# HSoumi/hybrid-als-twotower-recommender

Hardware: NVIDIA B200
Metric: als_ratings_per_sec_per_sweep (higher is better)
Workload: dtype f32

## Files before the change

### hybrid-als-twotower-recommender_b200/csrc/als_ws64.cu

```cuda
#include <cuda_bf16.h>

#include <cstdlib>

#include "als_ws_common.cuh"

namespace hals {
namespace ws64 {
using namespace ws;

constexpr int K = 64;
constexpr int kStageBytes = stage_bytes(K);
#ifndef HALS_WS_STAGES
#define HALS_WS_STAGES 10
#endif
constexpr int kStages = HALS_WS_STAGES;
constexpr int kAcc = 4, kAccCols = 128;
constexpr int kSlots = 2;
constexpr int kLd = 68;
constexpr int kSlotBytes = 2 * 64 * kLd * 4 + 512;
constexpr int kSolvers = 9;
constexpr int kScratchBytes = 1536;
constexpr int kN = 80;
constexpr int kThreads = 512;
constexpr int kWarpSolver = 0, kWarpGather = 9, kWarpMma = 11, kWarpDrain = 12;
static_assert(kStages % 2 == 0, "the two gather warps own alternate stages");
static_assert(kWarpSolver + kSolvers == kWarpGather && kWarpDrain + 4 == kThreads / 32 && kWarpDrain % 4 == 0, "role map");

struct Bars {
  uint64_t st_full[kStages], st_free[kStages];
  uint64_t st_scaled[kStages];
  uint64_t acc_full[kAcc], acc_free[kAcc];
  uint64_t sol_full[kSolvers];
  uint64_t slot_free[kSlots];
};

__device__ __forceinline__ float sel4(float a, float b, float c, float d, int i) {
  return i == 0 ? a : i == 1 ? b : i == 2 ? c : d;
}

__device__ __noinline__ void gather_role(uint32_t stages, Bars* bars, uint8_t* gscratch, const Range* rg,
                                         const int32_t* __restrict__ colidx, const uint32_t* __restrict__ vals_hl,
                                         const float* __restrict__ vals_sc, const uint8_t* __restrict__ src_hl, int zero_row,
                                         const int64_t* __restrict__ chunk_pos, const int32_t* __restrict__ chunk_cnt,
                                         int gw, int lane) {
  const int t_sub = lane >> 4, piece = lane & 15;
  const uint32_t ring = umma::smem_u32(gscratch);
  const uint32_t mpos = ring + 2 * kBurst * 128;
  const uint32_t mcnt = mpos + 2 * kBurst * 8;
  const int64_t k_hi = rg->chunk_hi;
  int64_t kw = rg->chunk_lo + gw;
  auto load_window = [&](int64_t& p, int& c) {
    const int64_t k = kw + 2 * lane;
    p = 0; c = 0;
    if (k < k_hi) { p = __ldg(chunk_pos + k); c = __ldg(chunk_cnt + k); }
    kw += 64;
  };
  int64_t wpos, npos;
  int wcnt, ncnt;
  load_window(wpos, wcnt);
  load_window(npos, ncnt);
  int wb = 0;
  int ci[kBurst];
  auto fill = [&](int buf) {
    if (lane >= wb * kBurst && lane < (wb + 1) * kBurst) {
      const uint32_t e = (uint32_t)(buf * kBurst + lane - wb * kBurst);
      asm volatile("st.shared.b64 [%0], %1;\n" ::"r"(mpos + e * 8u), "l"(wpos) : "memory");
      asm volatile("st.shared.b32 [%0], %1;\n" ::"r"(mcnt + e * 4u), "r"(wcnt) : "memory");
    }
#pragma unroll
    for (int c = 0; c < kBurst; ++c) {
      const int64_t pos = __shfl_sync(0xffffffffu, wpos, wb * kBurst + c);
      const int cnt = __shfl_sync(0xffffffffu, wcnt, wb * kBurst + c);
      ci[c] = lane < cnt ? __ldg(colidx + pos + lane) : zero_row;
    }
    if (++wb == 32 / kBurst) {
      wb = 0;
      wpos = npos; wcnt = ncnt;
      load_window(npos, ncnt);
    }
  };
  auto stash = [&](int buf) {
#pragma unroll
    for (int c = 0; c < kBurst; ++c)
      sts32(ring + (uint32_t)((buf * kBurst + c) * 32 + (lane & 1) * 16 + (lane >> 1)) * 4u, __int_as_float(ci[c]));
    __syncwarp();
  };

  const uint32_t blk_off = piece < 8 ? 0u : (uint32_t)kBlk;
  uint32_t dsto[4];
#pragma unroll
  for (int i = 0; i < 4; ++i) {
    const int t = t_sub + 2 * i;
    dsto[i] = blk_off + (uint32_t)t * kRowBytes + (uint32_t)(((piece & 7) ^ (t & 7)) << 4);
  }
  const uint64_t srcb = reinterpret_cast<uint64_t>(src_hl) + (uint64_t)piece * 16u;
  const uint32_t rdst = 2 * kBlk + (uint32_t)lane * kRowBytes + (uint32_t)((lane & 7) << 4);
  const uint32_t sdst = 2 * kBlk + (uint32_t)lane * kRowBytes + (uint32_t)((7 ^ (lane & 7)) << 4);
  uint32_t g = 0, s = (uint32_t)gw, u = 0;
#ifdef HALS_WS_PROFILE
  long long w_free = 0, t_iss = 0, t_fill = 0;
#endif
  fill(0);
  stash(0);
  fill(1);
  for (int buf = 0;; buf ^= 1) {
    bool done = false;
#pragma unroll 1
    for (int c = 0; c < kBurst; ++c) {
      int cnt;
      asm volatile("ld.shared.b32 %0, [%1];\n" : "=r"(cnt) : "r"(mcnt + (uint32_t)(buf * kBurst + c) * 4u));
      if (cnt <= 0) { done = true; break; }
      int64_t pos;
      asm volatile("ld.shared.b64 %0, [%1];\n" : "=l"(pos) : "r"(mpos + (uint32_t)(buf * kBurst + c) * 8u));
      const uint32_t ir = ring + (uint32_t)((buf * kBurst + c) * 32 + t_sub * 16) * 4u;
      const float4 c0 = lds128(ir), c1 = lds128(ir + 16), c2 = lds128(ir + 32), c3 = lds128(ir + 48);
      if (u > 0) { WS_T0(); umma::mbar_wait(&bars->st_free[s], (u - 1) & 1); WS_ACC(w_free); }
      WS_T0();
      const uint32_t st = stages + s * kStageBytes;
      const float colf[16] = {c0.x, c0.y, c0.z, c0.w, c1.x, c1.y, c1.z, c1.w, c2.x, c2.y, c2.z, c2.w, c3.x, c3.y, c3.z, c3.w};
#pragma unroll
      for (int i = 0; i < KC / 2; ++i) {
        uint64_t src;
        asm("mad.wide.u32 %0, %1, 256, %2;\n" : "=l"(src) : "r"((uint32_t)__float_as_int(colf[i])), "l"(srcb));
        cp_async16_raw(st + dsto[i & 3] + (uint32_t)(i >> 2) * (8 * kRowBytes), src);
      }
      {
        const bool ok = lane < cnt;
        const uint32_t* rp = vals_hl + pos + (ok ? lane : 0);
        asm volatile("cp.async.ca.shared.global [%0], [%1], 4, %2;\n" ::"r"(st + rdst), "l"(rp), "r"(ok ? 4 : 0) : "memory");
        if (vals_sc != nullptr) {
          const float* sp = vals_sc + pos + (ok ? lane : 0);
          asm volatile("cp.async.ca.shared.global [%0], [%1], 4, %2;\n" ::"r"(st + sdst), "l"(sp), "r"(ok ? 4 : 0) : "memory");
        }
      }
      cp_async_mbar_arrive_noinc(&bars->st_full[s]);
      WS_ACC(t_iss);
      ++g;
      s += 2;
      if (s >= (uint32_t)kStages) { s -= kStages; ++u; }
    }
    if (done) break;
    WS_T0();
    stash(buf ^ 1);
    fill(buf);
    WS_ACC(t_fill);
  }
#ifdef HALS_WS_PROFILE
  if (lane == 0 && blockIdx.x == 1) printf("G%d: chunks %u wait_free %lld issue %lld fill %lld\n", gw, g, w_free, t_iss, t_fill);
#endif
}

__device__ __noinline__ void scaler_role(uint32_t stages, Bars* bars, const Range* rg, int lane) {
  scale_stages<K, kStages>(stages, bars, rg, lane);
}

__device__ __noinline__ void mma_role(uint32_t sbase, uint32_t tmem, Bars* bars, const Range* rg,
                                      const int32_t* __restrict__ chunk_cnt, bool scaled, int lane) {
  constexpr uint32_t idesc = umma::make_instr_desc(umma::kFmtBF16, true, true, 128, kN);
  uint64_t* const ready = scaled ? bars->st_scaled : bars->st_full;
  const int64_t k_lo = rg->chunk_lo, k_hi = rg->chunk_hi;
  uint32_t s = 0, su = 0, b = 0, bu = 0;
  bool first = true;
#ifdef HALS_WS_PROFILE
  long long w_acc = 0, w_full = 0, t_issue = 0;
#endif
  int wc = 0, nc = 0;
  if (k_lo + lane < k_hi) wc = __ldg(chunk_cnt + k_lo + lane);
  if (k_lo + 32 + lane < k_hi) nc = __ldg(chunk_cnt + k_lo + 32 + lane);
  const bool leader = elect_one();
  const uint64_t ad0 = umma::make_smem_desc(sbase, kBlk, 1024, umma::kSwizzle128B);
  const uint64_t bd0 = umma::make_smem_desc(sbase, 2 * kBlk, 1024, umma::kSwizzle128B);
  for (int64_t kb = k_lo; kb < k_hi; kb += 32) {
    const int nk = (int)(k_hi - kb < 32 ? k_hi - kb : 32);
    for (int i = 0; i < nk; ++i) {
      const int cnt = __shfl_sync(0xffffffffu, wc, i);
      if (leader) {
        if (first) {
          if (bu > 0) { WS_T0(); umma::mbar_wait(&bars->acc_free[b], (bu - 1) & 1); WS_ACC(w_acc); }
          umma::fence_after_sync();
        }
        { WS_T0(); umma::mbar_wait(&ready[s], su & 1); WS_ACC(w_full); }
        WS_T0();
        const uint32_t td = tmem + b * kAccCols;
        const uint64_t so = (uint64_t)((s * kStageBytes) >> 4);
#pragma unroll
        for (int ks = 0; ks < KC / 16; ++ks)
          umma::mma_bf16(td, ad0 + so + (uint64_t)(ks * 2048 >> 4), bd0 + so + (uint64_t)(ks * 2048 >> 4), idesc,
                         !(first && ks == 0));
        umma::commit(&bars->st_free[s]);
        if (cnt <= KC) umma::commit(&bars->acc_full[b]);
        WS_ACC(t_issue);
      }
      __syncwarp();
      first = cnt <= KC;
      if (first) { if (++b == (uint32_t)kAcc) { b = 0; ++bu; } }
      if (++s == (uint32_t)kStages) { s = 0; ++su; }
    }
    wc = nc;
    nc = 0;
    if (kb + 64 + lane < k_hi) nc = __ldg(chunk_cnt + kb + 64 + lane);
  }
#ifdef HALS_WS_PROFILE
  if (blockIdx.x == 1 && leader) printf("M: wait_acc_free %lld wait_stage_full %lld issue %lld\n", w_acc, w_full, t_issue);
#endif
}

__device__ __noinline__ void drain_role(uint32_t slots, uint32_t tmem, Bars* bars, const Range* rg, int nsolv, int tid) {
  const int warp = tid >> 5;
  const int64_t n_rows = rg->item_hi - rg->item_lo;
  uint32_t b = 0, bu = 0, sl = 0, slu = 0, sv = 0;
#ifdef HALS_WS_PROFILE
  long long w_acc = 0, w_slot = 0, t_ld = 0;
#endif
  for (int64_t it = 0; it < n_rows; ++it) {
    { WS_T0(); umma::mbar_wait(&bars->acc_full[b], bu & 1); WS_ACC(w_acc); }
    umma::fence_after_sync();
    const uint32_t ta = tmem + b * kAccCols + ((uint32_t)(warp * 32) << 16);
    float a[64], e[16];
    {
      WS_T0();
      umma::tmem_ld32(ta, a);
      umma::tmem_ld32(ta + 32, a + 32);
      umma::tmem_ld16(ta + 64, e);
      WS_ACC(t_ld);
    }
    umma::fence_before_sync();
    umma::mbar_arrive(&bars->acc_free[b]);
    if (slu > 0) { WS_T0(); umma::mbar_wait(&bars->slot_free[sl], (slu - 1) & 1); WS_ACC(w_slot); }
    const uint32_t sb = slots + sl * kSlotBytes;
    const int m = tid & 63;
    const uint32_t rowp = sb + (tid < 64 ? 0u : (uint32_t)(64 * kLd * 4)) + (uint32_t)m * (kLd * 4);
#pragma unroll
    for (int n = 0; n < 64; n += 4) sts128(rowp + n * 4, a[n], a[n + 1], a[n + 2], a[n + 3]);
    const uint32_t bp = sb + 2 * 64 * kLd * 4;
    if (tid < 64) sts32(bp + m * 4, e[0] + e[1]);
    else sts32(bp + 256 + m * 4, e[0]);
    umma::mbar_arrive(&bars->sol_full[sv]);
    if (++b == (uint32_t)kAcc) { b = 0; ++bu; }
    if (++sl == (uint32_t)kSlots) { sl = 0; ++slu; }
    if (++sv == (uint32_t)nsolv) sv = 0;
  }
#ifdef HALS_WS_PROFILE
  if (tid == 0 && blockIdx.x == 1) printf("D: wait_acc_full %lld tmem_ld %lld wait_slot_free %lld\n", w_acc, t_ld, w_slot);
#endif
}

template <int JR>
__device__ __forceinline__ void elim_block(f32x2 (&R)[36], f32x2& bb2, const uint32_t P, const uint32_t Y,
                                           const uint32_t DI, const int ti, const int tj, const int lane) {
  const uint32_t oW = (uint32_t)ti * 16u;
  const uint32_t oL = (uint32_t)(tj & 3) * 16u + (uint32_t)(tj >> 2) * 4u;
  const uint32_t oB = oW + (uint32_t)(tj >> 1) * 64u + (uint32_t)(tj & 1) * 8u;
  auto publish = [&](uint32_t Pn, bool own) {
    if (JR & 1) sts64_if(own, Pn + oW + (JR >> 1) * 64 + 8, R[tri(JR, JR)]);
#pragma unroll
    for (int q = (JR + 1) & ~1; q < 8; q += 2) sts128x2_if(own, Pn + oW + (q >> 1) * 64, R[tri(q, JR)], R[tri(q + 1, JR)]);
  };
  {
    publish(P, tj == 0);
    sts32_if(ti == 0 && tj == JR, Y + (uint32_t)(8 * JR) * 4u, lo2(bb2));
    sts32_if(lane == 0, DI + (uint32_t)(8 * JR) * 4u, -rcp_fast(lo2(R[tri(JR, JR)])));
    __syncwarp();
  }
  const bool below = tj > JR;
#pragma unroll 1
  for (int jm = 0; jm < 8; ++jm) {
    const int j = 8 * JR + jm;
    const uint32_t Pj = P + ((uint32_t)(jm & 1) << 8);
    f32x2 w[8];
    float l[8];
    if (JR & 1) w[JR] = lds64x2(Pj + oW + (JR >> 1) * 64 + 8);
#pragma unroll
    for (int q = (JR + 1) & ~1; q < 8; q += 2) lds128x2(Pj + oW + (q >> 1) * 64, w[q], w[q + 1]);
    const float ninv = lds32(DI + (uint32_t)j * 4u);
#pragma unroll
    for (int c = JR; c < 8; ++c) l[c] = lds32(Pj + oL + (c >> 1) * 64 + (c & 1) * 8);
    const float zj = lds32(Y + (uint32_t)j * 4u);
    const f32x2 wb = lds64x2(Pj + oB);
    const f32x2 ninv2 = pack2(ninv, ninv);
    const float lj = tj > jm ? l[JR] : 0.f;
    const f32x2 lj2 = pack2(lj, lj);
    w[JR] = fmul2(w[JR], ninv2);
    R[tri(JR, JR)] = ffma2(w[JR], lj2, R[tri(JR, JR)]);
    const int jn = jm + 1;
    const float ninv_n = -rcp_fast((jn & 4) ? hi2(R[tri(JR, JR)]) : lo2(R[tri(JR, JR)]));
#pragma unroll
    for (int q = JR + 1; q < 8; ++q) {
      w[q] = fmul2(w[q], ninv2);
      R[tri(q, JR)] = ffma2(w[q], lj2, R[tri(q, JR)]);
    }
    {
      const bool on = tj == JR;
      const bool act_lo = below || (on && ti > jm), act_hi = below || (on && ti + 4 > jm);
      const f32x2 mb = fmul2(wb, ninv2);
      bb2 = ffma2(pack2(act_lo ? lo2(mb) : 0.f, act_hi ? hi2(mb) : 0.f), pack2(zj, zj), bb2);
    }
    {
      const uint32_t Pn = P + ((uint32_t)(jn & 1) << 8);
      const bool own = (tj == jn);
      publish(Pn, own);
      sts32_if(tj == JR && ti == (jn & 3) && jn < 8, Y + (uint32_t)(j + 1) * 4u, (jn & 4) ? hi2(bb2) : lo2(bb2));
      sts32_if(own && ti == (jn & 3), DI + (uint32_t)(j + 1) * 4u, ninv_n);
      __syncwarp();
    }
#pragma unroll
    for (int c = JR + 1; c < 8; ++c) {
      const f32x2 l2 = pack2(l[c], l[c]);
#pragma unroll
      for (int q = c; q < 8; ++q) R[tri(q, c)] = ffma2(w[q], l2, R[tri(q, c)]);
    }
  }
}

template <int JR>
__device__ __forceinline__ void back_block(const f32x2 (&R)[36], f32x2 (&x2)[8], const uint32_t Y, const uint32_t DI,
                                           const uint32_t T, const uint32_t RH, const int ti, const int tj,
                                           const int lane, float& out0, float& out1) {
  f32x2 acc0 = 0ull, acc1 = 0ull;
#pragma unroll
  for (int q = JR + 1; q < 8; ++q) {
    if ((q - JR) & 1) acc0 = ffma2(R[tri(q, JR)], x2[q], acc0);
    else acc1 = ffma2(R[tri(q, JR)], x2[q], acc1);
  }
  float ext = (lo2(acc0) + hi2(acc0)) + (lo2(acc1) + hi2(acc1));
  ext += __shfl_xor_sync(0xffffffffu, ext, 8);
  ext += __shfl_xor_sync(0xffffffffu, ext, 16);
  const float rh = lds32(Y + (uint32_t)(8 * JR + tj) * 4u) - ext;
  sts32(T + (uint32_t)(ti * 8 + tj) * 4u, lo2(R[tri(JR, JR)]));
  sts32(T + (uint32_t)((ti + 4) * 8 + tj) * 4u, hi2(R[tri(JR, JR)]));
  sts32_if(ti == 0, RH + (uint32_t)tj * 4u, rh);
  __syncwarp();
  float r[8], di[8], xb[8];
  {
    const float4 a = lds128(RH), b = lds128(RH + 16);
    r[0] = a.x; r[1] = a.y; r[2] = a.z; r[3] = a.w; r[4] = b.x; r[5] = b.y; r[6] = b.z; r[7] = b.w;
    const float4 c = lds128(DI + (uint32_t)(8 * JR) * 4u), d = lds128(DI + (uint32_t)(8 * JR) * 4u + 16);
    di[0] = c.x; di[1] = c.y; di[2] = c.z; di[3] = c.w; di[4] = d.x; di[5] = d.y; di[6] = d.z; di[7] = d.w;
  }
#pragma unroll
  for (int e = 7; e >= 0; --e) {
    xb[e] = -r[e] * di[e];
    if (e > 0) {
      float t[8];
      const float4 a = lds128(T + (uint32_t)(e * 8) * 4u);
      t[0] = a.x; t[1] = a.y; t[2] = a.z; t[3] = a.w;
      if (e > 4) {
        const float4 b = lds128(T + (uint32_t)(e * 8 + 4) * 4u);
        t[4] = b.x; t[5] = b.y; t[6] = b.z; t[7] = b.w;
      }
#pragma unroll
      for (int c = 0; c < e; ++c) r[c] = fmaf(-t[c], xb[e], r[c]);
    }
  }
  __syncwarp();
  x2[JR] = pack2(sel4(xb[0], xb[1], xb[2], xb[3], ti), sel4(xb[4], xb[5], xb[6], xb[7], ti));
  if ((lane >> 2) == JR) {
    const int e2 = lane & 3;
    out0 = sel4(xb[0], xb[2], xb[4], xb[6], e2);
    out1 = sel4(xb[1], xb[3], xb[5], xb[7], e2);
  }
}

__device__ __forceinline__ void eliminate(f32x2 (&R)[36], f32x2& bb2, const uint32_t P, const uint32_t Y, const uint32_t DI,
                                          int ti, int tj, int lane) {
  elim_block<0>(R, bb2, P, Y, DI, ti, tj, lane);
  elim_block<1>(R, bb2, P, Y, DI, ti, tj, lane);
  elim_block<2>(R, bb2, P, Y, DI, ti, tj, lane);
  elim_block<3>(R, bb2, P, Y, DI, ti, tj, lane);
  elim_block<4>(R, bb2, P, Y, DI, ti, tj, lane);
  elim_block<5>(R, bb2, P, Y, DI, ti, tj, lane);
  elim_block<6>(R, bb2, P, Y, DI, ti, tj, lane);
  elim_block<7>(R, bb2, P, Y, DI, ti, tj, lane);
  __syncwarp();
}
__device__ __forceinline__ void back_store(const f32x2 (&R)[36], const uint32_t Y, const uint32_t DI, const uint32_t T,
                                           const uint32_t RH, int ti, int tj, int lane, float* __restrict__ dst,
                                           __nv_bfloat16* __restrict__ dst_hl, int row) {
  f32x2 x2[8];
#pragma unroll
  for (int q = 0; q < 8; ++q) x2[q] = 0ull;
  float out0 = 0.f, out1 = 0.f;
  back_block<7>(R, x2, Y, DI, T, RH, ti, tj, lane, out0, out1);
  back_block<6>(R, x2, Y, DI, T, RH, ti, tj, lane, out0, out1);
  back_block<5>(R, x2, Y, DI, T, RH, ti, tj, lane, out0, out1);
  back_block<4>(R, x2, Y, DI, T, RH, ti, tj, lane, out0, out1);
  back_block<3>(R, x2, Y, DI, T, RH, ti, tj, lane, out0, out1);
  back_block<2>(R, x2, Y, DI, T, RH, ti, tj, lane, out0, out1);
  back_block<1>(R, x2, Y, DI, T, RH, ti, tj, lane, out0, out1);
  back_block<0>(R, x2, Y, DI, T, RH, ti, tj, lane, out0, out1);
  *reinterpret_cast<float2*>(dst + (int64_t)row * K + 2 * lane) = make_float2(out0, out1);
  if (dst_hl) {
    const __nv_bfloat162 h = __floats2bfloat162_rn(out0, out1);
    const __nv_bfloat162 l = __floats2bfloat162_rn(out0 - __low2float(h), out1 - __high2float(h));
    __nv_bfloat162* o = reinterpret_cast<__nv_bfloat162*>(dst_hl + (int64_t)row * (2 * K));
    o[lane] = h;
    o[K / 2 + lane] = l;
  }
}

__device__ __noinline__ void solver_role(uint32_t slots, uint32_t scratch, Bars* bars, float* __restrict__ dst,
                                         __nv_bfloat16* __restrict__ dst_hl, float* __restrict__ workspace, float reg,
                                         const int32_t* __restrict__ item_row, const int32_t* __restrict__ item_len,
                                         const int32_t* __restrict__ item_slot, const float* __restrict__ gram_tiles,
                                         const Range* rg, int nsolv, int w, int lane) {
  const int ti = lane >> 3, tj = lane & 7;
  const uint32_t P = scratch, Y = P + 512, DI = Y + 256, T = DI + 256, RH = T + 256;
  const int64_t n_items = rg->item_hi;
#ifdef HALS_WS_PROFILE
  long long w_slot = 0, t_load = 0, t_elim = 0, t_back = 0;
  int n_solved = 0;
#endif
  int64_t it = rg->item_lo + w;
  int row_n = 0, len_n = 0, slot_n = -1;
  if (it < n_items) { row_n = __ldg(item_row + it); len_n = __ldg(item_len + it); slot_n = __ldg(item_slot + it); }
  uint32_t mine = 0;
  for (uint32_t i = (uint32_t)w; it < n_items; i += nsolv, it += nsolv, ++mine) {
    const int row = row_n, len = len_n, wslot = slot_n;
    {
      const int64_t nx = it + nsolv;
      if (nx < n_items) { row_n = __ldg(item_row + nx); len_n = __ldg(item_len + nx); slot_n = __ldg(item_slot + nx); }
    }
    const uint32_t sl = i % kSlots;
    { WS_T0(); umma::mbar_wait(&bars->sol_full[w], mine & 1); WS_ACC(w_slot); }
    const uint32_t S1 = slots + sl * kSlotBytes, S2 = S1 + 64 * kLd * 4, B1 = S2 + 64 * kLd * 4, B2 = B1 + 256;
    if (wslot >= 0) {
      float* W = workspace + (size_t)wslot * ((size_t)K * K + K + 4);
      for (int e = lane; e < K * K; e += 32) {
        const int m = e >> 6, n = e & 63;
        W[e] = lds32(S1 + (uint32_t)(m * kLd + n) * 4u) + lds32(S2 + (uint32_t)(m * kLd + n) * 4u) +
               lds32(S2 + (uint32_t)(n * kLd + m) * 4u);
      }
      W[K * K + lane] = lds32(B1 + lane * 4) + lds32(B2 + lane * 4);
      W[K * K + 32 + lane] = lds32(B1 + (32 + lane) * 4) + lds32(B2 + (32 + lane) * 4);
      if (lane == 0) W[K * K + K] = (float)len;
      __syncwarp();
      if (lane == 0) umma::mbar_arrive(&bars->slot_free[sl]);
      continue;
    }
    f32x2 R[36];
    f32x2 bb2;
    {
      WS_T0();
      const float lam = reg * (float)len;
      const uint32_t p1 = S1 + (uint32_t)(ti * kLd + tj) * 4u, p2 = S2 + (uint32_t)(ti * kLd + tj) * 4u;
      const uint32_t pt = S2 + (uint32_t)(tj * kLd + ti) * 4u;
#pragma unroll
      for (int q = 0; q < 8; ++q) {
#pragma unroll
        for (int c = 0; c <= q; ++c) {
          float v[2];
#pragma unroll
          for (int h = 0; h < 2; ++h) {
            const uint32_t mn = (uint32_t)((8 * q + 4 * h) * kLd + 8 * c) * 4u, nm = (uint32_t)(8 * c * kLd + 8 * q + 4 * h) * 4u;
            v[h] = lds32(p1 + mn) + lds32(p2 + mn) + lds32(pt + nm);
            if (q == c) v[h] += (ti + 4 * h == tj) ? lam : 0.f;
          }
          R[tri(q, c)] = pack2(v[0], v[1]);
        }
      }
      if (gram_tiles != nullptr) {
        const float4* gp = reinterpret_cast<const float4*>(gram_tiles) + lane * 18;
#pragma unroll
        for (int i = 0; i < 18; ++i) {
          const float4 g = __ldg(gp + i);
          R[2 * i] = ffma2(pack2(g.x, g.y), pack2(1.f, 1.f), R[2 * i]);
          R[2 * i + 1] = ffma2(pack2(g.z, g.w), pack2(1.f, 1.f), R[2 * i + 1]);
        }
      }
      const uint32_t ob = (uint32_t)(ti + 8 * tj) * 4u;
      bb2 = pack2(lds32(B1 + ob) + lds32(B2 + ob), lds32(B1 + ob + 16) + lds32(B2 + ob + 16));
      __syncwarp();
      if (lane == 0) umma::mbar_arrive(&bars->slot_free[sl]);
      WS_ACC(t_load);
    }
    {
      WS_T0();
      eliminate(R, bb2, P, Y, DI, ti, tj, lane);
      WS_ACC(t_elim);
    }
    {
      WS_T0();
      back_store(R, Y, DI, T, RH, ti, tj, lane, dst, dst_hl, row);
      WS_ACC(t_back);
    }
#ifdef HALS_WS_PROFILE
    ++n_solved;
#endif
  }
#ifdef HALS_WS_PROFILE
  if (lane == 0 && blockIdx.x == 1)
    printf("S%d: solved %d wait_slot %lld load %lld elim %lld back %lld\n", w, n_solved, w_slot, t_load, t_elim, t_back);
#endif
}

__global__ void __launch_bounds__(kThreads, 1)
als_ws64_kernel(const int32_t* __restrict__ colidx, const uint32_t* __restrict__ vals_hl,
                const float* __restrict__ vals_sc, const float* __restrict__ gram_tiles,
                const __nv_bfloat16* __restrict__ src_hl, float* __restrict__ dst, float reg,
                const int32_t* __restrict__ item_row, const int32_t* __restrict__ item_len,
                const int32_t* __restrict__ item_slot, const int64_t* __restrict__ item_chunk0,
                const int64_t* __restrict__ item_cost0, const int64_t* __restrict__ chunk_pos,
                const int32_t* __restrict__ chunk_cnt, int64_t n_items, int zero_row, float* __restrict__ workspace,
                __nv_bfloat16* __restrict__ dst_hl) {
  extern __shared__ uint8_t smem_dyn[];
  __shared__ Bars bars;
  __shared__ Range range;
  __shared__ uint32_t tmem_slot;
  uint8_t* base = reinterpret_cast<uint8_t*>((reinterpret_cast<uintptr_t>(smem_dyn) + 1023) & ~uintptr_t(1023));
  const int tid = threadIdx.x, warp = tid >> 5, lane = tid & 31;
  if (warp == kWarpDrain) umma::tmem_alloc(&tmem_slot, kAcc * kAccCols);
  if (tid == 32) {
    for (int s = 0; s < kStages; ++s) {
      umma::mbar_init(&bars.st_full[s], 32);
      umma::mbar_init(&bars.st_free[s], 1);
      umma::mbar_init(&bars.st_scaled[s], 1);
    }
    for (int b = 0; b < kAcc; ++b) { umma::mbar_init(&bars.acc_full[b], 1); umma::mbar_init(&bars.acc_free[b], 128); }
    for (int s = 0; s < kSlots; ++s) umma::mbar_init(&bars.slot_free[s], 1);
    for (int s = 0; s < kSolvers; ++s) umma::mbar_init(&bars.sol_full[s], 128);
    umma::mbar_fence_init();
  }
  if (tid < 2) cta_range(&range, item_cost0, item_chunk0, n_items, tid);
  zero_r_blocks<K, kStages, kThreads>(base, tid);
  umma::fence_proxy_async();
  umma::fence_before_sync();
  __syncthreads();
  umma::fence_after_sync();
  const uint32_t tmem = tmem_slot;
  const uint32_t sbase = umma::smem_u32(base);
#ifdef HALS_WS_PROFILE
  const long long t_cta0 = clock64();
#endif
  const uint32_t slots = sbase + kStages * kStageBytes;
  const uint32_t scratch = slots + kSlots * kSlotBytes;
  uint8_t* gscratch = base + kStages * kStageBytes + kSlots * kSlotBytes + kSolvers * kScratchBytes;

  const bool implicit = vals_sc != nullptr;
  const int nsolv = implicit ? kSolvers - 1 : kSolvers;
  if (warp >= kWarpDrain) {
    drain_role(slots, tmem, &bars, &range, nsolv, tid - kWarpDrain * 32);
  } else if (warp >= kWarpGather && warp < kWarpMma) {
    gather_role(sbase, &bars, gscratch + (warp - kWarpGather) * kGatherScratch, &range, colidx, vals_hl, vals_sc,
                reinterpret_cast<const uint8_t*>(src_hl), zero_row, chunk_pos, chunk_cnt, warp - kWarpGather, lane);
  } else if (warp == kWarpMma) {
    mma_role(sbase, tmem, &bars, &range, chunk_cnt, implicit, lane);
  } else if (warp - kWarpSolver < nsolv) {
    solver_role(slots, scratch + (uint32_t)(warp - kWarpSolver) * kScratchBytes, &bars, dst, dst_hl, workspace, reg, item_row,
                item_len, item_slot, gram_tiles, &range, nsolv, warp - kWarpSolver, lane);
  } else {
    scaler_role(sbase, &bars, &range, lane);
  }
#ifdef HALS_WS_PROFILE
  const long long t_role = clock64() - t_cta0;
#endif
  umma::fence_before_sync();
  __syncthreads();
#ifdef HALS_WS_PROFILE
  if (lane == 0 && (warp == kWarpDrain || warp == kWarpGather || warp == kWarpMma || warp == kWarpSolver))
    printf("C %d w%d role %lld cta %lld\n", (int)blockIdx.x, warp, t_role, clock64() - t_cta0);
#endif
  if (warp == kWarpDrain) umma::tmem_dealloc(tmem, kAcc * kAccCols);
}

__global__ void __launch_bounds__(128)
als_reduce_solve64_warp_kernel(const float* __restrict__ workspace, float* __restrict__ dst,
                               __nv_bfloat16* __restrict__ dst_hl, float reg, const int32_t* __restrict__ long_row,
                               const int32_t* __restrict__ long_slot0, const int32_t* __restrict__ long_nseg,
                               const float* __restrict__ gram) {
  constexpr int SF = K * K + K + 4;
  __shared__ __align__(16) float sA[SF];
  __shared__ __align__(16) uint8_t sScratch[kScratchBytes];
  const int tid = threadIdx.x, lane = tid & 31;
  const int row = long_row[blockIdx.x];
  const int s0 = long_slot0[blockIdx.x], ns = long_nseg[blockIdx.x];
  const int stride = slot_final_stride(ns);
  for (int e = tid * 4; e < SF; e += 128 * 4) {
    float4 acc = make_float4(0.f, 0.f, 0.f, 0.f);
    for (int q = 0; q < ns; q += stride) {
      const float4 v = *reinterpret_cast<const float4*>(workspace + (size_t)(s0 + q) * SF + e);
      acc.x += v.x; acc.y += v.y; acc.z += v.z; acc.w += v.w;
    }
    *reinterpret_cast<float4*>(sA + e) = acc;
  }
  __syncthreads();
  if (tid >= 32) return;
  const int ti = lane >> 3, tj = lane & 7;
  const float lam = reg * sA[K * K + K];
  f32x2 R[36];
#pragma unroll
  for (int q = 0; q < 8; ++q) {
#pragma unroll
    for (int c = 0; c <= q; ++c) {
      float v[2];
#pragma unroll
      for (int h = 0; h < 2; ++h) {
        const int m = ti + 4 * h + 8 * q, n = tj + 8 * c;
        v[h] = sA[m * K + n] + (m == n ? lam : 0.f) + (gram != nullptr ? __ldg(gram + m * K + n) : 0.f);
      }
      R[tri(q, c)] = pack2(v[0], v[1]);
    }
  }
  f32x2 bb2 = pack2(sA[K * K + ti + 8 * tj], sA[K * K + ti + 4 + 8 * tj]);
  const uint32_t P = umma::smem_u32(sScratch), Y = P + 512, DI = Y + 256, T = DI + 256, RH = T + 256;
  eliminate(R, bb2, P, Y, DI, ti, tj, lane);
  back_store(R, Y, DI, T, RH, ti, tj, lane, dst, dst_hl, row);
}

}

__global__ void gram_to_tiles64_kernel(const float* __restrict__ G, float* __restrict__ tiles) {
  const int lane = threadIdx.x, ti = lane >> 3, tj = lane & 7;
  for (int q = 0; q < 8; ++q)
    for (int c = 0; c <= q; ++c)
      for (int h = 0; h < 2; ++h)
        tiles[lane * 72 + ws64::tri(q, c) * 2 + h] = G[(ti + 4 * h + 8 * q) * ws64::K + tj + 8 * c];
}

int als_half_step_ws64(const int32_t* colidx, const uint32_t* vals_hl, const float* src, int64_t n_src, float* dst,
                       float reg, const hals_als_plan* plan, float* slots, void* split_buf, void* dst_hl,
                       const float* gram, float* gram_tiles, cudaStream_t st) {
  using namespace ws64;
  __nv_bfloat16* hl = reinterpret_cast<__nv_bfloat16*>(split_buf);
  HALS_REQUIRE(n_src < (int64_t)1 << 31, "at most 2^31 - 1 source rows");
  if (src != nullptr) {
    if (int rc = als_launch_split_bf16(src, n_src, K, hl, st)) return rc;
    HALS_CUDA(cudaMemsetAsync(hl + (size_t)n_src * 2 * K, 0, 4 * K, st));
  }
  const size_t smem = (size_t)kStages * kStageBytes + (size_t)kSlots * kSlotBytes + (size_t)kSolvers * kScratchBytes +
                      2 * kGatherScratch + 1024;
  static_assert(kStages * kStageBytes + kSlots * kSlotBytes + kSolvers * kScratchBytes + 2 * kGatherScratch + 1024 <= 227 * 1024 - 1024,
                "shared memory budget");
  HALS_CUDA(cudaFuncSetAttribute(als_ws64_kernel, cudaFuncAttributeMaxDynamicSharedMemorySize, (int)smem));
  const bool implicit = gram != nullptr;
  if (implicit) {
    HALS_REQUIRE(plan->vals_scale && plan->item_npos && gram_tiles, "implicit mode needs the plan's vals_scale / item_npos");
    gram_to_tiles64_kernel<<<1, 32, 0, st>>>(gram, gram_tiles);
    HALS_LAUNCH_CHECK();
  }
  int64_t grid = sm_count();
  if (grid > plan->n_items) grid = plan->n_items;
  als_ws64_kernel<<<(unsigned)grid, kThreads, smem, st>>>(colidx, vals_hl, implicit ? plan->vals_scale : nullptr,
                                                         implicit ? gram_tiles : nullptr, hl, dst, reg, plan->item_row,
                                                         implicit ? plan->item_npos : plan->item_len, plan->item_slot, plan->item_chunk0, plan->item_cost0,
                                                         plan->chunk_pos, plan->chunk_cnt, plan->n_items, (int)n_src, slots,
                                                         reinterpret_cast<__nv_bfloat16*>(dst_hl));
  HALS_LAUNCH_CHECK();
  if (plan->n_long_rows > 0) {
    if (int rc = als_launch_slot_group_sum(slots, plan, K * K + K + 4, st)) return rc;
    als_reduce_solve64_warp_kernel<<<(unsigned)plan->n_long_rows, 128, 0, st>>>(
        slots, dst, reinterpret_cast<__nv_bfloat16*>(dst_hl), reg, plan->long_row, plan->long_slot0, plan->long_nseg, gram);
    HALS_LAUNCH_CHECK();
  }
  return 0;
}

}
```

Baseline: 6.218 billion.

## Replace round-robin solver assignment with dynamic ticket queue

Solver warps stop taking fixed round-robin items. Each one now draws tickets from a shared atomic counter and publishes its warp id in a small shared queue. The drain warps look up the owner of each row in that queue before signalling it, so a solver that finishes early (for example on short rows) can take the next item instead of waiting behind slower peers. The cost is an atomic and shuffle per item, a volatile spin-wait in the drain path, and item metadata loads that are no longer prefetched as far ahead.

```diff
diff --git a/hybrid-als-twotower-recommender_b200/csrc/als_ws64.cu b/hybrid-als-twotower-recommender_b200/csrc/als_ws64.cu
--- a/hybrid-als-twotower-recommender_b200/csrc/als_ws64.cu
+++ b/hybrid-als-twotower-recommender_b200/csrc/als_ws64.cu
@@ -32,7 +32,23 @@
   uint64_t acc_full[kAcc], acc_free[kAcc];
   uint64_t sol_full[kSolvers];
   uint64_t slot_free[kSlots];
+  uint32_t ticket;
+  uint32_t queue[16];
 };
+constexpr uint32_t kQueue = 16;
+static_assert(kQueue >= kSolvers, "one outstanding ticket per solver");
+
+__device__ __forceinline__ uint32_t ticket_owner(const uint32_t* e, uint32_t t) {
+  const volatile uint32_t* q = e;
+  uint32_t v = *q;
+  if ((v >> 4) == t) return v & 15u;
+  const long long t0 = clock64();
+  while (((v = *q) >> 4) != t) {
+    __nanosleep(100);
+    if (clock64() - t0 > 4000000000ll) __trap();
+  }
+  return v & 15u;
+}
 
 __device__ __forceinline__ float sel4(float a, float b, float c, float d, int i) {
   return i == 0 ? a : i == 1 ? b : i == 2 ? c : d;
@@ -205,10 +221,10 @@
 #endif
 }
 
-__device__ __noinline__ void drain_role(uint32_t slots, uint32_t tmem, Bars* bars, const Range* rg, int nsolv, int tid) {
+__device__ __noinline__ void drain_role(uint32_t slots, uint32_t tmem, Bars* bars, const Range* rg, int tid) {
   const int warp = tid >> 5;
   const int64_t n_rows = rg->item_hi - rg->item_lo;
-  uint32_t b = 0, bu = 0, sl = 0, slu = 0, sv = 0;
+  uint32_t b = 0, bu = 0, sl = 0, slu = 0;
 #ifdef HALS_WS_PROFILE
   long long w_acc = 0, w_slot = 0, t_ld = 0;
 #endif
@@ -235,10 +251,9 @@
     const uint32_t bp = sb + 2 * 64 * kLd * 4;
     if (tid < 64) sts32(bp + m * 4, e[0] + e[1]);
     else sts32(bp + 256 + m * 4, e[0]);
-    umma::mbar_arrive(&bars->sol_full[sv]);
+    umma::mbar_arrive(&bars->sol_full[ticket_owner(&bars->queue[it % kQueue], (uint32_t)it)]);
     if (++b == (uint32_t)kAcc) { b = 0; ++bu; }
     if (++sl == (uint32_t)kSlots) { sl = 0; ++slu; }
-    if (++sv == (uint32_t)nsolv) sv = 0;
   }
 #ifdef HALS_WS_PROFILE
   if (tid == 0 && blockIdx.x == 1) printf("D: wait_acc_full %lld tmem_ld %lld wait_slot_free %lld\n", w_acc, t_ld, w_slot);
@@ -402,7 +417,7 @@
                                          __nv_bfloat16* __restrict__ dst_hl, float* __restrict__ workspace, float reg,
                                          const int32_t* __restrict__ item_row, const int32_t* __restrict__ item_len,
                                          const int32_t* __restrict__ item_slot, const float* __restrict__ gram_tiles,
-                                         const Range* rg, int nsolv, int w, int lane) {
+                                         const Range* rg, int w, int lane) {
   const int ti = lane >> 3, tj = lane & 7;
   const uint32_t P = scratch, Y = P + 512, DI = Y + 256, T = DI + 256, RH = T + 256;
   const int64_t n_items = rg->item_hi;
@@ -410,16 +425,26 @@
   long long w_slot = 0, t_load = 0, t_elim = 0, t_back = 0;
   int n_solved = 0;
 #endif
-  int64_t it = rg->item_lo + w;
+  uint32_t i_n;
+  int64_t it_n;
   int row_n = 0, len_n = 0, slot_n = -1;
-  if (it < n_items) { row_n = __ldg(item_row + it); len_n = __ldg(item_len + it); slot_n = __ldg(item_slot + it); }
-  uint32_t mine = 0;
-  for (uint32_t i = (uint32_t)w; it < n_items; i += nsolv, it += nsolv, ++mine) {
+  auto draw = [&]() {
+    uint32_t t = 0;
+    if (lane == 0)
+      asm volatile("atom.shared.add.u32 %0, [%1], 1;\n" : "=r"(t) : "r"(umma::smem_u32(&bars->ticket)) : "memory");
+    i_n = __shfl_sync(0xffffffffu, t, 0);
+    it_n = rg->item_lo + i_n;
+    if (it_n < n_items) {
+      if (lane == 0)
+        asm volatile("st.volatile.shared.u32 [%0], %1;\n" ::"r"(umma::smem_u32(&bars->queue[i_n % kQueue])),
+                     "r"((i_n << 4) | (uint32_t)w) : "memory");
+      row_n = __ldg(item_row + it_n); len_n = __ldg(item_len + it_n); slot_n = __ldg(item_slot + it_n);
+    }
+  };
+  draw();
+  for (uint32_t mine = 0; it_n < n_items; ++mine) {
+    const uint32_t i = i_n;
     const int row = row_n, len = len_n, wslot = slot_n;
-    {
-      const int64_t nx = it + nsolv;
-      if (nx < n_items) { row_n = __ldg(item_row + nx); len_n = __ldg(item_len + nx); slot_n = __ldg(item_slot + nx); }
-    }
     const uint32_t sl = i % kSlots;
     { WS_T0(); umma::mbar_wait(&bars->sol_full[w], mine & 1); WS_ACC(w_slot); }
     const uint32_t S1 = slots + sl * kSlotBytes, S2 = S1 + 64 * kLd * 4, B1 = S2 + 64 * kLd * 4, B2 = B1 + 256;
@@ -435,6 +460,7 @@
       if (lane == 0) W[K * K + K] = (float)len;
       __syncwarp();
       if (lane == 0) umma::mbar_arrive(&bars->slot_free[sl]);
+      draw();
       continue;
     }
     f32x2 R[36];
@@ -478,6 +504,7 @@
       eliminate(R, bb2, P, Y, DI, ti, tj, lane);
       WS_ACC(t_elim);
     }
+    draw();
     {
       WS_T0();
       back_store(R, Y, DI, T, RH, ti, tj, lane, dst, dst_hl, row);
@@ -516,6 +543,8 @@
       umma::mbar_init(&bars.st_scaled[s], 1);
     }
     for (int b = 0; b < kAcc; ++b) { umma::mbar_init(&bars.acc_full[b], 1); umma::mbar_init(&bars.acc_free[b], 128); }
+    bars.ticket = 0;
+    for (uint32_t q = 0; q < kQueue; ++q) bars.queue[q] = ~0u;
     for (int s = 0; s < kSlots; ++s) umma::mbar_init(&bars.slot_free[s], 1);
     for (int s = 0; s < kSolvers; ++s) umma::mbar_init(&bars.sol_full[s], 128);
     umma::mbar_fence_init();
@@ -538,7 +567,7 @@
   const bool implicit = vals_sc != nullptr;
   const int nsolv = implicit ? kSolvers - 1 : kSolvers;
   if (warp >= kWarpDrain) {
-    drain_role(slots, tmem, &bars, &range, nsolv, tid - kWarpDrain * 32);
+    drain_role(slots, tmem, &bars, &range, tid - kWarpDrain * 32);
   } else if (warp >= kWarpGather && warp < kWarpMma) {
     gather_role(sbase, &bars, gscratch + (warp - kWarpGather) * kGatherScratch, &range, colidx, vals_hl, vals_sc,
                 reinterpret_cast<const uint8_t*>(src_hl), zero_row, chunk_pos, chunk_cnt, warp - kWarpGather, lane);
@@ -546,7 +575,7 @@
     mma_role(sbase, tmem, &bars, &range, chunk_cnt, implicit, lane);
   } else if (warp - kWarpSolver < nsolv) {
     solver_role(slots, scratch + (uint32_t)(warp - kWarpSolver) * kScratchBytes, &bars, dst, dst_hl, workspace, reg, item_row,
-                item_len, item_slot, gram_tiles, &range, nsolv, warp - kWarpSolver, lane);
+                item_len, item_slot, gram_tiles, &range, warp - kWarpSolver, lane);
   } else {
     scaler_role(sbase, &bars, &range, lane);
   }
```

New measurement: 5.429 billion, median of 6. -12.7%, worse.
